# genome/bam-readcount

Measured on AMD Instinct MI355X. Metric: pileup base-events/sec, higher is better.
Workload: dtype u32+f32

## Files before the change

bam_readcount_amd/csrc/brc_engine.hip:

```cpp
#include <hip/hip_runtime.h>
#include <atomic>
#include <chrono>

#include <stdio.h>
#include <stdlib.h>
#include <string.h>

#include <algorithm>
#include <string>
#include <mutex>
#include <vector>

#include "brc_host.h"

namespace brc {

struct Counters {
    unsigned long long n_events, n_positions, w_sm, w_nm, w_lib;
    unsigned int n_indel_slots, n_xev;
    unsigned int xev_max, n_wave_reads;
    unsigned int n_wave_big, n_wave_huge;
    unsigned int n_literal, n_wave_eqx;
    unsigned int n_wave_eqx_big, pad_;
};
// ... 1797 lines not shown

static void* pinned_alloc(size_t n) {
    void* p = nullptr;
    if (hipHostMalloc(&p, n ? n : 1, hipHostMallocDefault) != hipSuccess) return nullptr;
    return p;
}
static void pinned_release(void* p) { (void)hipHostFree(p); }
static const HostAlloc kPinned = {pinned_alloc, pinned_release};

static std::atomic<uint64_t> g_dev_allocs{0}, g_dev_alloc_ns{0};
struct DBuf {
    void* p = nullptr; size_t cap = 0;
    size_t req = 0;
    hipError_t ensure(size_t bytes) {
        req = bytes;
        if (bytes <= cap) return hipSuccess;
        struct Tm { std::chrono::steady_clock::time_point t0 = std::chrono::steady_clock::now();
                    ~Tm() { g_dev_alloc_ns += (uint64_t)std::chrono::duration_cast<std::chrono::nanoseconds>(std::chrono::steady_clock::now() - t0).count(); ++g_dev_allocs; } } tm_;
        const bool regrow = p != nullptr;
        if (p) { (void)hipFree(p); p = nullptr; cap = 0; }
        size_t want = bytes + (regrow ? bytes / 2 : bytes / 8) + 256;
        hipError_t e = hipMalloc(&p, want);
        if (e != hipSuccess) { e = hipMalloc(&p, bytes); want = bytes; }
        if (e == hipSuccess) cap = want;
        return e;
    }
    void release() { if (p) (void)hipFree(p); p = nullptr; cap = 0; }
};

enum { T_ANNOTATE = 0, T_SCAN_ENDS, T_TILES, T_PILEUP, T_COUNT, T_INDEL_SCAN, T_INDEL_FILL, T_INDEL_REDUCE, T_N };
static const char* kKernelNames[BRC_NKERNEL] = {"k_annotate", "k_scan_ends", "k_tiles", "k_pileup", "k_xev_fold+finalize",
                                                "k_scan_indel", "k_indel_fill", "k_indel_reduce"};

#define HIPCHK(x) do { hipError_t _e = (x); if (_e != hipSuccess) { return hip_fail(_e, #x); } } while (0)

class HipBackend : public Backend {
    std::string err;
    int device = 0;
    hipStream_t stream = nullptr;
    enum { EV_RING = 32 };
    struct EvSet { hipEvent_t evt[T_N + 1]; hipEvent_t ev_indel[4]; };
    std::vector<EvSet> evsets;
    hipEvent_t* evt = nullptr;
    bool have_events = false;
    DevCfg c; DevIn in;
    int64_t ntiles = 0; uint64_t n_indel_cap = 0;
    std::vector<int64_t> lib_base;
    DBuf d_pos, d_flag, d_mapq, d_lib, d_lq, d_nc, d_co, d_so, d_qo, d_nm, d_sm, d_tags, d_cigar, d_seq, d_qual, d_ref, d_refcode;
    std::vector<uint16_t> h_wanted; bool has_wanted = false; DBuf d_wanted; std::vector<uint32_t> h_tilelist; DBuf d_tilelist;
    HBuf<Staged::WidePair> h_wpairs; unsigned wide_slices = 1;
    DBuf d_wpairs;
    DBuf d_bq, d_bqw, d_bqrow, d_pieceoff, d_pieces, d_rare, d_keyreach, d_libbase, d_reads, d_agg, d_rng, d_ncol, d_depth, d_slotid, d_si, d_sf, d_xev, d_xevc, d_xevn, d_unavail, d_cnt, d_cursor, d_ev, d_evraw, d_ievoff, d_iout, d_ctr, d_tilectr, d_part, d_wavelist, d_nc_k1;
    DBuf d_tlen, d_toff, d_text, d_tctx, d_total64, d_lastproc;
    DBuf d_xcnt, d_xend, d_xidx, d_xagg;
    HBuf<char> h_text[2]; HBuf<uint32_t> h_toff[2]; HBuf<uint32_t> h_total;
    hipStream_t stream2 = nullptr; hipEvent_t ev_text[2] = {nullptr, nullptr}, ev_lines = nullptr;
    hipStream_t stream3 = nullptr; hipEvent_t* ev_indel = nullptr; DBuf d_agg2;
    bool text_started[2] = {false, false}; uint64_t text_total[2] = {0, 0}; int64_t text_n[2] = {0, 0}; int text_slot = 0;
    Planes pl_last;
    enum { COMPACT_PIECES_PER_READ = 12 };
    bool compact_on = false; uint64_t compact_total = 0; bool compact_sized = false;
    bool wave_on = false;
    bool wave_big = false;
    enum { WAVE_FORM_BLOCKS = 768,
           WAVE_FORM_BLOCKS_BIG = 512,
           WAVE_FORM_BLOCKS_HUGE = 256 };
    bool wave_huge = false;
    bool wave_eqx = false; uint32_t s_max_ncigar = 0;
    bool cursor_on = false;
    unsigned long long h_steps[3] = {0, 0, 0};
    DBuf d_ccnt, d_coff, d_cpieces, d_crare, d_crng, d_ctot;
    HBuf<uint32_t> h_ncol, h_depth, h_slotid, h_si, h_unavail; HBuf<float> h_sf; HBuf<IndelOut> h_iout; HBuf<XAgg> h_xagg; HBuf<uint32_t> h_lastproc[2];
    std::vector<XAgg> xagg_compact;
    size_t xev_cap = 0;
    enum { XEV_SHARDS = 1024 };
    std::vector<IndelOut> iout_compact;
    Counters h_ctr;
    bool computed = false;
#ifdef BRC_CHECKED
    DBuf d_chk; ChkState h_chk;
    void chk_fill() {
        memset(&h_chk, 0, sizeof h_chk);
        auto set = [&](int b, const DBuf& d) { h_chk.ext[b].lo = (uint64_t)d.p; h_chk.ext[b].hi = (uint64_t)d.p + d.req; };
        set(CB_CIGAR, d_cigar); set(CB_SEQ, d_seq); set(CB_QUAL, d_qual); set(CB_REFCODE, d_refcode); set(CB_EB, d_bq); set(CB_BQW, d_bqw);
        set(CB_PIECES, d_pieces); set(CB_RARE, d_rare); set(CB_KEYREACH, d_keyreach); set(CB_READS, d_reads); set(CB_EVRAW, d_evraw); set(CB_CNT, d_cnt);
        set(CB_WANTED, d_wanted); set(CB_RNG, d_rng); set(CB_UNAVAIL, d_unavail); set(CB_TILELIST, d_tilelist); set(CB_NCOL, d_ncol); set(CB_DEPTH, d_depth);
        set(CB_SLOTID, d_slotid); set(CB_SI, d_si); set(CB_SF, d_sf); set(CB_XEV, d_xev); set(CB_XEVN, d_xevn); set(CB_TILECTR, d_tilectr);
        const bool cz = compact_on && compact_sized;
        set(CB_KP_PIECES, cz ? d_cpieces : d_pieces); set(CB_KP_RARE, cz ? d_crare : d_rare); set(CB_KP_RNG, cz ? d_crng : d_rng);
        if (const char* sh = getenv("BRC_CHECKED_SHRINK")) { const int b = atoi(sh); const char* cpos = strchr(sh, ':'); if (b >= 0 && b < CB_N && cpos) { const uint64_t by = strtoull(cpos + 1, nullptr, 10); ChkExt& x = h_chk.ext[b]; x.hi = x.hi - x.lo > by ? x.hi - by : x.lo; } }
// ... 20 lines not shown
        err = b;
        return e == hipErrorOutOfMemory ? BRC_E_NOMEM : BRC_E_HIP;
    }

  public:
    int init(int dev) {
        int n = 0;
        if (hipGetDeviceCount(&n) != hipSuccess || n <= 0) { err = "no HIP device visible"; return BRC_E_NODEVICE; }
        if (dev < 0 || dev >= n) { err = "device ordinal out of range"; return BRC_E_NODEVICE; }
        device = dev;
        HIPCHK(hipSetDevice(device));
        HIPCHK(hipStreamCreateWithFlags(&stream, hipStreamNonBlocking));
        { const int rc0 = ensure_evsets(1); if (rc0) return rc0; }
        HIPCHK(hipStreamCreateWithFlags(&stream2, hipStreamNonBlocking));
        HIPCHK(hipStreamCreateWithFlags(&stream3, hipStreamNonBlocking));
        {
            uint32_t* d_bad = nullptr; uint32_t bad = 0;
            HIPCHK(hipMalloc(&d_bad, sizeof(uint32_t)));
            HIPCHK(hipMemsetAsync(d_bad, 0, sizeof(uint32_t), stream));
            hipLaunchKernelGGL(k_divcheck, dim3((DIV_SMALL_N * DIV_SMALL_M + 255) / 256), dim3(256), 0, stream, d_bad);
            HIPCHK(hipMemcpyAsync(&bad, d_bad, sizeof(uint32_t), hipMemcpyDeviceToHost, stream));
            HIPCHK(hipStreamSynchronize(stream));
            (void)hipFree(d_bad);
            if (bad) { err = "this device's reciprocal does not give correctly rounded small-integer quotients (div_small self-check failed)"; return BRC_E_HIP; }
        }
        for (int i = 0; i < 2; ++i) { HIPCHK(hipEventCreateWithFlags(&ev_text[i], hipEventDisableTiming)); h_text[i].A = &kPinned; h_toff[i].A = &kPinned; }
        HIPCHK(hipEventCreateWithFlags(&ev_lines, hipEventDisableTiming));
        h_total.A = &kPinned;
        h_ncol.A = h_depth.A = h_slotid.A = h_si.A = h_unavail.A = &kPinned; h_sf.A = &kPinned; h_iout.A = &kPinned; h_xagg.A = &kPinned; h_wpairs.A = &kPinned; h_lastproc[0].A = h_lastproc[1].A = &kPinned;
        return BRC_OK;
    }
    ~HipBackend() override {
        (void)hipSetDevice(device);
        if (getenv("BRC_ENGINE_TIMING")) fprintf(stderr, "device buffers: %llu (re)allocations, %.3f s\n", (unsigned long long)g_dev_allocs.load(), (double)g_dev_alloc_ns.load() * 1e-9);
        DBuf* all[] = {&d_pos, &d_flag, &d_mapq, &d_lib, &d_lq, &d_nc, &d_co, &d_so, &d_qo, &d_nm, &d_sm, &d_tags, &d_cigar, &d_seq, &d_qual,
                       &d_ref, &d_refcode, &d_bq, &d_bqw, &d_bqrow, &d_pieceoff, &d_pieces, &d_rare, &d_keyreach, &d_libbase, &d_reads, &d_agg, &d_rng, &d_ncol, &d_depth, &d_slotid, &d_si, &d_sf, &d_xev, &d_xevc, &d_xevn, &d_unavail, &d_cnt,
                       &d_cursor, &d_ev, &d_evraw, &d_ievoff, &d_iout, &d_ctr, &d_tilectr, &d_part, &d_tlen, &d_toff, &d_text, &d_tctx, &d_total64, &d_lastproc, &d_xcnt, &d_xend, &d_xidx, &d_xagg, &d_wanted, &d_tilelist, &d_wavelist, &d_nc_k1, &d_wpairs};
        for (DBuf* b : all) b->release();
        d_ccnt.release(); d_coff.release(); d_cpieces.release(); d_crare.release(); d_crng.release(); d_ctot.release();
#ifdef BRC_CHECKED
        d_chk.release();
#endif
        for (int i = 0; i < 2; ++i) { h_text[i].destroy(); h_toff[i].destroy(); if (ev_text[i]) (void)hipEventDestroy(ev_text[i]); }
        h_total.destroy();
        if (ev_lines) (void)hipEventDestroy(ev_lines);
        if (stream2) (void)hipStreamDestroy(stream2);
        if (stream3) (void)hipStreamDestroy(stream3);
        d_agg2.release();
        h_ncol.destroy(); h_depth.destroy(); h_slotid.destroy(); h_si.destroy(); h_unavail.destroy(); h_sf.destroy(); h_iout.destroy(); h_xagg.destroy(); h_wpairs.destroy(); h_lastproc[0].destroy(); h_lastproc[1].destroy();
        if (w_init) { w_ncol.destroy(); w_depth.destroy(); w_slotid.destroy(); w_si.destroy(); w_unavail.destroy(); w_sf.destroy(); }
        for (EvSet& es : evsets) { for (int i = 0; i <= T_N; ++i) if (es.evt[i]) (void)hipEventDestroy(es.evt[i]); for (int i = 0; i < 4; ++i) if (es.ev_indel[i]) (void)hipEventDestroy(es.ev_indel[i]); }
        if (stream) (void)hipStreamDestroy(stream);
    }
    int ensure_evsets(size_t n) {
        while (evsets.size() < n) {
            EvSet es; memset(&es, 0, sizeof es);
            evsets.push_back(es);
            for (int i = 0; i <= T_N; ++i) HIPCHK(hipEventCreate(&evsets.back().evt[i]));
            for (int i = 0; i < 4; ++i) HIPCHK(hipEventCreate(&evsets.back().ev_indel[i]));
        }
        evt = evsets[0].evt; ev_indel = evsets[0].ev_indel; have_events = true;
        return BRC_OK;
    }
    const HostAlloc* host_alloc() override { return &kPinned; }
    const char* last_error() const override { return err.c_str(); }

    template <class T>
    int up(DBuf& d, const HBuf<T>& h, size_t n) {
        HIPCHK(d.ensure((n + 16) * sizeof(T)));
        if (n) HIPCHK(hipMemcpyAsync(d.p, h.p, n * sizeof(T), hipMemcpyHostToDevice, stream));
        return BRC_OK;
    }

    int up_arena(DBuf& d, const HBuf<uint8_t>& h, const std::vector<Staged::Seg>& segs, uint64_t total) {
        if (segs.empty()) return up(d, h, h.n);
        HIPCHK(d.ensure((size_t)total + 16));
        for (const Staged::Seg& g : segs) if (g.n) HIPCHK(hipMemcpyAsync((uint8_t*)d.p + g.off, g.p, (size_t)g.n, hipMemcpyHostToDevice, stream));
        return BRC_OK;
    }
    bool adopts_arenas() const override { return true; }

    int upload(const brc_config& cfg, const Staged& s, Geometry& g) override {
        HIPCHK(hipSetDevice(device));
        computed = false;
        memset(&c, 0, sizeof c);
        c.min_mapq = cfg.min_mapq; c.min_bq = cfg.min_bq; c.per_lib = cfg.per_lib; c.insertion_centric = cfg.insertion_centric;
        c.Lp = g.Lp; c.ref_len_check = cfg.ref_len_check; c.has_ref = g.ref != nullptr;
        g.PS = (g.P + 63) & ~(int64_t)63;
        c.beg0 = g.beg0; c.end = g.end; c.pos0 = g.pos0; c.P = g.P; c.PS = g.PS; c.ref_lo = g.ref_lo; c.ref_hi = g.ref_hi; c.ref_len = g.ref_len;
        c.n_reads = s.n; c.table_len = test_knob(TK_NO_TABLE) ? 0 : s.modal_len();
        c.n_pieces = s.n_pieces; lib_base = s.lib_base; c.max_lqseq = s.max_lqseq;
        c.ibucket_shift = indel_bucket_shift(s.n_indel_ops, c.P, c.Lp);
        if (const char* ib = test_knob(TK_IBUCKET_SHIFT)) { const int v = atoi(ib); if (v == 2 || v == 4 || v == 6) c.ibucket_shift = v; }
        choose_pack(s.max_lqseq, test_knob(TK_FLUSH_K) ? atoi(test_knob(TK_FLUSH_K)) : 0, test_knob(TK_PACK_LIM) ? atoi(test_knob(TK_PACK_LIM)) : 0, c.flush_k, c.pack_lim, c.pack_lim_lo, c.pack_shift);
// ... 94 lines not shown
        HIPCHK(d_ctr.ensure(sizeof(Counters))); HIPCHK(d_tilectr.ensure(((size_t)ntiles * Lp + 1) * sizeof(uint4)));
        in.iev_off = nullptr;
        if (n_indel_cap) {
            const size_t nbk = (size_t)indel_buckets(c);
            if ((rc = up(d_ievoff, s.iev_off, n))) return rc;
            in.iev_off = (const uint32_t*)d_ievoff.p;
            HIPCHK(d_cnt.ensure(nbk * 4 + 16)); HIPCHK(d_cursor.ensure(nbk * 4 + 16)); HIPCHK(d_evraw.ensure((n_indel_cap + 1) * sizeof(IndelEv)));
            HIPCHK(d_ev.ensure((n_indel_cap + 1) * sizeof(IndelEv))); HIPCHK(d_iout.ensure((n_indel_cap + 1) * sizeof(IndelOut)));
        }
        if (has_wanted && P) {
            HIPCHK(hipMemsetAsync(d_ncol.p, 0, Lp * P * 4, stream)); HIPCHK(hipMemsetAsync(d_depth.p, 0, Lp * P * 4, stream));
            HIPCHK(hipMemsetD32Async((hipDeviceptr_t)d_slotid.p, (int)((uint32_t)NB_NONE | ((uint32_t)NB_NONE << 8)), Lp * P, stream));
            HIPCHK(hipMemsetAsync(d_tilectr.p, 0, (size_t)ntiles * Lp * sizeof(uint4), stream));
        }
        HIPCHK(hipStreamSynchronize(stream));
        return BRC_OK;
    }

    template <class Op, bool INCL>
    int scan(const typename Op::T* src, typename Op::T* dst, int64_t n) { return scan_on<Op, INCL>(src, dst, n, stream, d_agg); }
    template <class Op, bool INCL>
    int scan_on(const typename Op::T* src, typename Op::T* dst, int64_t n, hipStream_t st, DBuf& scratch) {
        if (n <= 0) return BRC_OK;
        const int64_t nb = (n + SCAN_CHUNK - 1) / SCAN_CHUNK;
        typename Op::T* agg = (typename Op::T*)scratch.p;
        hipLaunchKernelGGL((k_scan_reduce<Op>), dim3((unsigned)nb), dim3(SCAN_T), 0, st, src, n, agg);
        hipLaunchKernelGGL((k_scan_aggregates<Op>), dim3(1), dim3(1024), 0, st, agg, nb);
        hipLaunchKernelGGL((k_scan_apply<Op, INCL>), dim3((unsigned)nb), dim3(SCAN_T), 0, st, src, dst, n, (const typename Op::T*)agg);
        HIPCHK(hipGetLastError());
        return BRC_OK;
    }

    int enqueue_pass(size_t set) {
        evt = evsets[set].evt; ev_indel = evsets[set].ev_indel;
        const int64_t n = c.n_reads, P = c.P; const int Lp = c.Lp;
        int rc;
        Counters* ctr = (Counters*)d_ctr.p;
        lists_host = false;
        HIPCHK(hipMemsetAsync(ctr, 0, sizeof(Counters), stream));
        HIPCHK(hipMemsetAsync(d_xevn.p, 0, (size_t)XEV_SHARDS * XEV_CTR_STRIDE * 4, stream));
        const bool indels = n_indel_cap > 0 && P > 0 && n > 0;
        const int64_t n_buckets = indel_buckets(c);
        if (indels) HIPCHK(hipMemsetAsync(d_cnt.p, 0, (size_t)n_buckets * 4, stream));
#ifdef BRC_CHECKED
        if (set == 0) { chk_fill(); HIPCHK(hipMemcpyAsync(d_chk.p, &h_chk, sizeof h_chk, hipMemcpyHostToDevice, stream)); HIPCHK(hipStreamSynchronize(stream)); }
#endif
        Planes pl = {(uint32_t*)d_ncol.p, (uint32_t*)d_depth.p, (uint32_t*)d_slotid.p, (uint32_t*)d_si.p, (float*)d_sf.p, (uint32_t*)d_unavail.p,
                     (XEv*)d_xev.p, (uint32_t*)d_xevn.p, (uint32_t)xev_cap, (uint32_t)XEV_SHARDS};
        pl_last = pl;
        const DRead* reads = (const DRead*)d_reads.p;
        HIPCHK(hipEventRecord(evt[T_ANNOTATE], stream));
        if (n > 0) {
            const int64_t rl = c.ref_hi - c.ref_lo;
            if (c.has_ref)
                hipLaunchKernelGGL(k_refcode, dim3((unsigned)(((rl + 2 * REFCODE_PAD + 15) / 16 + 255) / 256)), dim3(256), 0, stream, in.ref, (uint8_t*)d_refcode.p, rl);
            if (h_wpairs.n)
                hipLaunchKernelGGL(k_wide_rows, dim3((unsigned)((h_wpairs.n + 255) / 256), wide_slices), dim3(256), 0, stream, c, in, (const uint2*)d_wpairs.p, (uint32_t)h_wpairs.n, (uint16_t*)in.bqw);
            DevIn in_k1 = in;
            if (wave_on || cursor_on) {
                hipLaunchKernelGGL(k_pick_wave, dim3((unsigned)((n + 255) / 256)), dim3(256), 0, stream, c, in, (uint32_t*)d_nc_k1.p, (uint32_t*)d_wavelist.p, (uint32_t)n, &ctr->n_wave_reads, &ctr->n_wave_big, &ctr->n_wave_huge,
                                   wave_on ? 1 : 0, cursor_on ? 1 : 0, &ctr->n_literal, &ctr->n_wave_eqx, &ctr->n_wave_eqx_big);
                in_k1.n_cigar = (const uint32_t*)d_nc_k1.p;
            }
            {
#define BRC_LAUNCH_K1(OS, SH) hipLaunchKernelGGL((k_annotate_groups<OS, SH>), dim3((unsigned)((n + 255) / 256)), dim3(256), 0, stream, c, in_k1, (DRead*)d_reads.p, (const uint32_t*)d_pieceoff.p, \
                                   (Piece*)d_pieces.p, (PieceRare*)d_rare.p, (int2*)d_keyreach.p,                                                                               \
                                   (uint8_t*)in.eb, indels ? (IndelEv*)d_evraw.p : (IndelEv*)nullptr, (uint32_t*)d_cnt.p,                                    \
                                   in.cigar, in.qual, in.seq4, (const uint8_t*)d_refcode.p + REFCODE_PAD, has_wanted ? (const uint16_t*)d_wanted.p : (const uint16_t*)nullptr)
                if (Lp == 1) { if (c.pack_shift == 16) BRC_LAUNCH_K1(true, 16); else BRC_LAUNCH_K1(true, 12); }
                else { if (c.pack_shift == 16) BRC_LAUNCH_K1(false, 16); else BRC_LAUNCH_K1(false, 12); }
#undef BRC_LAUNCH_K1
                if (wave_on) {
                    const unsigned nb = (unsigned)std::min<int64_t>((n + 3) / 4, (int64_t)WAVE_FORM_BLOCKS);
#define BRC_LAUNCH_K1W(SH, MCAP, WAVES, GRID, LIST, STEP, COUNT) hipLaunchKernelGGL((k_annotate_wave<SH, MCAP, WAVES>), dim3(GRID), dim3(WAVES * 64), 0, stream, c, in, LIST, STEP, (const unsigned int*)(COUNT),     \
                                   (DRead*)d_reads.p, (const uint32_t*)d_pieceoff.p, (Piece*)d_pieces.p, (PieceRare*)d_rare.p, (int2*)d_keyreach.p,                                   \
                                   (uint8_t*)in.eb, indels ? (IndelEv*)d_evraw.p : (IndelEv*)nullptr, (uint32_t*)d_cnt.p,                                          \
                                   (const uint8_t*)d_refcode.p + REFCODE_PAD, has_wanted ? (const uint16_t*)d_wanted.p : (const uint16_t*)nullptr)
                    const uint32_t* const wl = (const uint32_t*)d_wavelist.p;
                    if (c.pack_shift == 16) BRC_LAUNCH_K1W(16, AW_MCAP, 4, nb, wl, 1, &ctr->n_wave_reads); else BRC_LAUNCH_K1W(12, AW_MCAP, 4, nb, wl, 1, &ctr->n_wave_reads);
                    if (wave_big) {
                        const unsigned nbb = (unsigned)std::min<int64_t>(n, (int64_t)WAVE_FORM_BLOCKS_BIG);
                        if (c.pack_shift == 16) BRC_LAUNCH_K1W(16, AW_MCAP_BIG, 1, nbb, wl + (n - 1), -1, &ctr->n_wave_big); else BRC_LAUNCH_K1W(12, AW_MCAP_BIG, 1, nbb, wl + (n - 1), -1, &ctr->n_wave_big);
                    }
                    if (wave_eqx) {
#define BRC_LAUNCH_K1E(SH, MCAP, WAVES, GRID, LIST, STEP, COUNT) hipLaunchKernelGGL((k_annotate_wave<SH, MCAP, WAVES, true>), dim3(GRID), dim3(WAVES * 64), 0, stream, c, in, LIST, STEP, (const unsigned int*)(COUNT),     \
                                   (DRead*)d_reads.p, (const uint32_t*)d_pieceoff.p, (Piece*)d_pieces.p, (PieceRare*)d_rare.p, (int2*)d_keyreach.p,                                   \
                                   (uint8_t*)in.eb, indels ? (IndelEv*)d_evraw.p : (IndelEv*)nullptr, (uint32_t*)d_cnt.p,                                          \
                                   (const uint8_t*)d_refcode.p + REFCODE_PAD, has_wanted ? (const uint16_t*)d_wanted.p : (const uint16_t*)nullptr)
                        if (c.pack_shift == 16) BRC_LAUNCH_K1E(16, AW_MCAP_EQX, 4, nb, wl + (3 * n + 48), 1, &ctr->n_wave_eqx); else BRC_LAUNCH_K1E(12, AW_MCAP_EQX, 4, nb, wl + (3 * n + 48), 1, &ctr->n_wave_eqx);
                        if (s_max_ncigar > (uint32_t)AW_MCAP_EQX) {
                            const unsigned nbe = (unsigned)std::min<int64_t>(n, (int64_t)WAVE_FORM_BLOCKS_BIG);
                            if (c.pack_shift == 16) BRC_LAUNCH_K1E(16, AW_MCAP_EQX_BIG, 1, nbe, wl + (4 * n + 47), -1, &ctr->n_wave_eqx_big); else BRC_LAUNCH_K1E(12, AW_MCAP_EQX_BIG, 1, nbe, wl + (4 * n + 47), -1, &ctr->n_wave_eqx_big);
                        }
#undef BRC_LAUNCH_K1E
                    }
                    if (wave_huge) {
                        const unsigned nbh = (unsigned)std::min<int64_t>(n, (int64_t)WAVE_FORM_BLOCKS_HUGE);
                        if (c.pack_shift == 16) BRC_LAUNCH_K1W(16, AW_MCAP_HUGE, 1, nbh, wl + (n + 16), 1, &ctr->n_wave_huge); else BRC_LAUNCH_K1W(12, AW_MCAP_HUGE, 1, nbh, wl + (n + 16), 1, &ctr->n_wave_huge);
                    }
#undef BRC_LAUNCH_K1W
                }
                if (cursor_on) {
                    const unsigned nbc = (unsigned)std::min<int64_t>((n + 63) / 64, 1024);
#define BRC_LAUNCH_K1C(SH) hipLaunchKernelGGL((k_annotate_cursor<SH>), dim3(nbc), dim3(64), 0, stream, c, in, (const uint32_t*)d_wavelist.p + (2 * (size_t)n + 32), (const unsigned int*)&ctr->n_literal,    \
                                   (DRead*)d_reads.p, (const uint32_t*)d_pieceoff.p, (Piece*)d_pieces.p, (PieceRare*)d_rare.p, (int2*)d_keyreach.p, (uint8_t*)in.eb,                     \
                                   indels ? (IndelEv*)d_evraw.p : (IndelEv*)nullptr, (uint32_t*)d_cnt.p, has_wanted ? (const uint16_t*)d_wanted.p : (const uint16_t*)nullptr)
                    if (c.pack_shift == 16) BRC_LAUNCH_K1C(16); else BRC_LAUNCH_K1C(12);
#undef BRC_LAUNCH_K1C
                }
            }
            if (c.per_lib) {
                HIPCHK(hipMemsetAsync(d_unavail.p, 0xff, (size_t)c.PS * 4, stream));
                hipLaunchKernelGGL(k_unavail, dim3((unsigned)((n + 255) / 256)), dim3(256), 0, stream, c, in, (uint32_t*)d_unavail.p);
            }
        } else if (c.per_lib && P > 0) HIPCHK(hipMemsetAsync(d_unavail.p, 0xff, (size_t)c.PS * 4, stream));
        HIPCHK(hipEventRecord(evt[T_SCAN_ENDS], stream));
#ifdef BRC_EXP_KNOBS
        static const bool indel_overlap = getenv("BRC_INDEL_OVERLAP") && atoi(getenv("BRC_INDEL_OVERLAP")) != 0;
#else
        const bool indel_overlap = false;
#endif
        auto launch_indel = [&](hipStream_t si, DBuf& scratch) -> int {
            HIPCHK(hipEventRecord(ev_indel[0], si));
            int r2;
            if ((r2 = scan_on<OpSumU32, false>((const uint32_t*)d_cnt.p, (uint32_t*)d_cursor.p, n_buckets, si, scratch))) return r2;
            HIPCHK(hipEventRecord(ev_indel[1], si));
            hipLaunchKernelGGL(k_indel_scatter, dim3((unsigned)((n_indel_cap + 255) / 256)), dim3(256), 0, si, c, (const IndelEv*)d_evraw.p, (int64_t)n_indel_cap,
                               (uint32_t*)d_cursor.p, (IndelEv*)d_ev.p);
            HIPCHK(hipEventRecord(ev_indel[2], si));
            hipLaunchKernelGGL(k_indel_reduce, dim3((unsigned)std::min<int64_t>((n_buckets + 255) / 256, 4096)), dim3(256), 0, si, c, in, reads,
                               (const uint32_t*)d_cnt.p, (const uint32_t*)d_cursor.p, n_buckets, (IndelEv*)d_ev.p, (const uint32_t*)d_unavail.p,
                               (IndelOut*)d_iout.p, ctr);
            HIPCHK(hipEventRecord(ev_indel[3], si));
            return BRC_OK;
        };
        if (indels && indel_overlap) {
            HIPCHK(hipStreamWaitEvent(stream3, evt[T_SCAN_ENDS], 0));
            if ((rc = launch_indel(stream3, d_agg2))) return rc;
        }
        const int64_t np_all = c.n_pieces;
        const int64_t trb = (np_all + TR_CHUNK - 1) / TR_CHUNK;
        if (np_all > 0 && ntiles > 0) {
            hipLaunchKernelGGL(k_reach_blockmax, dim3((unsigned)trb), dim3(TR_T), 0, stream, (const int2*)d_keyreach.p, np_all, (const int64_t*)d_libbase.p, Lp, (unsigned long long*)d_agg.p);
            hipLaunchKernelGGL((k_scan_aggregates<OpMaxU64>), dim3(1), dim3(1024), 0, stream, (unsigned long long*)d_agg.p, trb);
        }
        HIPCHK(hipEventRecord(evt[T_TILES], stream));
        for (int l = 0; l < Lp && ntiles > 0; ++l)
            if (lib_base[(size_t)l + 1] == lib_base[(size_t)l]) HIPCHK(hipMemsetAsync((uint2*)d_rng.p + (int64_t)l * ntiles, 0, (size_t)ntiles * sizeof(uint2), stream));
        if (np_all > 0 && ntiles > 0)
            hipLaunchKernelGGL(k_tiles_all, dim3((unsigned)trb), dim3(TR_T), 0, stream, c, (const int2*)d_keyreach.p, np_all, (const int64_t*)d_libbase.p, Lp,
                               (const unsigned long long*)d_agg.p, ntiles, (uint2*)d_rng.p);
        const int64_t n_listed = (int64_t)h_tilelist.size();
        if (has_wanted && n_listed > 0)
            hipLaunchKernelGGL(k_narrow_tiles, dim3((unsigned)((n_listed * Lp + 255) / 256)), dim3(256), 0, stream, (const uint16_t*)d_wanted.p, (const uint32_t*)d_tilelist.p, n_listed, ntiles, Lp, c.pos0,
                               (uint2*)d_rng.p, (const int2*)d_keyreach.p);
        const uint4* kp_pieces = (const uint4*)d_pieces.p; const PieceRare* kp_rare = (const PieceRare*)d_rare.p; const uint2* kp_rng = (const uint2*)d_rng.p;
        if (compact_on && ntiles > 0 && np_all > 0) {
            const size_t nslot = (size_t)ntiles * (size_t)Lp;
            HIPCHK(d_ccnt.ensure((nslot + 2) * 4)); HIPCHK(d_coff.ensure((nslot + 2) * 4)); HIPCHK(d_crng.ensure((nslot + 1) * sizeof(uint2))); HIPCHK(d_ctot.ensure(24));
            HIPCHK(hipMemsetAsync(d_ctot.p, 0, 24, stream));
            HIPCHK(hipMemsetAsync((uint32_t*)d_ccnt.p + nslot, 0, 4, stream));
            const dim3 cg((unsigned)((ntiles + 3) / 4), (unsigned)Lp);
            const bool by_read = Lp == 1 && !(test_knob(TK_COMPACT) && atoi(test_knob(TK_COMPACT)) == 2);
            if (by_read) {
                HIPCHK(hipMemsetAsync(d_ccnt.p, 0, nslot * 4, stream));
                hipLaunchKernelGGL(k_count_piece_tiles, dim3((unsigned)((np_all + 255) / 256)), dim3(256), 0, stream, c, (const uint4*)d_pieces.p, np_all, (uint32_t*)d_ccnt.p);
            }
            else
            hipLaunchKernelGGL((k_compact_tiles<true>), cg, dim3(256), 0, stream, c, (const uint4*)d_pieces.p, (const PieceRare*)d_rare.p, (const uint2*)d_rng.p, ntiles,
                               (uint32_t*)d_ccnt.p, (const uint32_t*)nullptr, (uint4*)nullptr, (PieceRare*)nullptr, (uint2*)nullptr, (unsigned long long*)d_ctot.p);
            if ((rc = scan<OpSumU32, false>((const uint32_t*)d_ccnt.p, (uint32_t*)d_coff.p, (int64_t)nslot + 1))) return rc;
            const bool first_pass = !compact_sized;
            if (!compact_sized) {
                uint32_t tot = 0;
                HIPCHK(hipMemcpyAsync(&tot, (const uint32_t*)d_coff.p + nslot, 4, hipMemcpyDeviceToHost, stream));
                HIPCHK(hipMemcpyAsync(h_steps, d_ctot.p, 16, hipMemcpyDeviceToHost, stream));
                HIPCHK(hipStreamSynchronize(stream));
                compact_total = tot; compact_sized = true;
                HIPCHK(d_cpieces.ensure(((size_t)compact_total + 4) * sizeof(Piece))); HIPCHK(d_crare.ensure(((size_t)compact_total + 2) * sizeof(PieceRare)));
            }
            if (by_read)
                hipLaunchKernelGGL(k_compact_reads, dim3((unsigned)((ntiles + 4 * CR_GROUP - 1) / (4 * CR_GROUP))), dim3(256), 0, stream, c, (const uint4*)d_pieces.p, (const PieceRare*)d_rare.p, (const uint2*)d_rng.p, (const uint32_t*)d_pieceoff.p, (const int2*)d_keyreach.p, ntiles,
                                   (const uint32_t*)d_coff.p, (uint4*)d_cpieces.p, (PieceRare*)d_crare.p, (uint2*)d_crng.p, (unsigned long long*)d_ctot.p);
            else
            hipLaunchKernelGGL((k_compact_tiles<false>), cg, dim3(256), 0, stream, c, (const uint4*)d_pieces.p, (const PieceRare*)d_rare.p, (const uint2*)d_rng.p, ntiles,
                               (uint32_t*)d_ccnt.p, (const uint32_t*)d_coff.p, (uint4*)d_cpieces.p, (PieceRare*)d_crare.p, (uint2*)d_crng.p, (unsigned long long*)d_ctot.p);
            if (by_read && first_pass) {
                HIPCHK(hipMemcpyAsync(h_steps, d_ctot.p, 24, hipMemcpyDeviceToHost, stream));
                HIPCHK(hipStreamSynchronize(stream));
                if (h_steps[2]) { err = "tile compaction: a tile holds more live read segments than the pass over the segments counted for it"; return BRC_E_HIP; }
            }
            kp_pieces = (const uint4*)d_cpieces.p; kp_rare = (const PieceRare*)d_crare.p; kp_rng = (const uint2*)d_crng.p;
#ifdef BRC_CHECKED
            {
                HIPCHK(hipStreamSynchronize(stream));
                ChkState seen; HIPCHK(hipMemcpy(&seen, d_chk.p, sizeof seen, hipMemcpyDeviceToHost));
                chk_fill(); ChkState upd = h_chk; upd.count = seen.count; upd.kernel = seen.kernel; upd.site = seen.site; upd.buf = seen.buf; upd.addr = seen.addr; upd.bytes = seen.bytes; upd.unit = seen.unit; upd.piece = seen.piece;
                HIPCHK(hipMemcpy(d_chk.p, &upd, sizeof upd, hipMemcpyHostToDevice));
            }
#endif
        }
        HIPCHK(hipEventRecord(evt[T_PILEUP], stream));
        if (ntiles > 0) {
            unsigned nwg = (unsigned)(((has_wanted ? n_listed : ntiles) + PILEUP_WAVES - 1) / PILEUP_WAVES);
            nwg = (nwg + 7u) & ~7u;
#ifdef BRC_EXP_KNOBS
            static const unsigned dyn_lds = getenv("BRC_PILEUP_LDS_PAD") ? (unsigned)atoi(getenv("BRC_PILEUP_LDS_PAD")) : 0u;
#else
            const unsigned dyn_lds = 0u;
#endif
#define BRC_LAUNCH_KP(W, SH) hipLaunchKernelGGL((k_pileup2<W, SH>), dim3(nwg, (unsigned)Lp), dim3(PILEUP_WAVES * 64), dyn_lds, stream, c, in, kp_pieces, kp_rare, \
                               kp_rng, ntiles, pl, (uint4*)d_tilectr.p, in.eb, in.bqw, (const uint32_t*)d_unavail.p,                                                     \
                               (const uint8_t*)d_refcode.p + REFCODE_PAD, (const uint16_t*)d_wanted.p, (const uint32_t*)d_tilelist.p, n_listed)
            if (has_wanted) { if (n_listed > 0) { if (c.pack_shift == 16) BRC_LAUNCH_KP(true, 16); else BRC_LAUNCH_KP(true, 12); } }
            else { if (c.pack_shift == 16) BRC_LAUNCH_KP(false, 16); else BRC_LAUNCH_KP(false, 12); }
#undef BRC_LAUNCH_KP
        }
        HIPCHK(hipEventRecord(evt[T_COUNT], stream));
        if (ntiles > 0) {
            const int64_t nxb = ntiles * Lp;
            HIPCHK(hipMemsetAsync(d_xcnt.p, 0, (size_t)nxb * 4, stream));
            hipLaunchKernelGGL(k_xev_compact, dim3((unsigned)XEV_SHARDS), dim3(256), 0, stream, (const XEv*)d_xev.p, (const uint32_t*)d_xevn.p, (uint32_t)xev_cap,
                               (uint32_t)XEV_SHARDS, (XEv*)d_xevc.p, ctr, (uint32_t*)d_xcnt.p, Lp);
            if ((rc = scan<OpSumU32, false>((const uint32_t*)d_xcnt.p, (uint32_t*)d_xend.p, nxb))) return rc;
            hipLaunchKernelGGL(k_xev_scatter, dim3(256), dim3(256), 0, stream, (const XEv*)d_xevc.p, (const Counters*)ctr, (uint32_t*)d_xend.p, (uint32_t*)d_xidx.p, Lp);
            hipLaunchKernelGGL(k_xev_fold, dim3((unsigned)std::min<int64_t>((nxb + 255) / 256, 2048)), dim3(256), 0, stream, (const XEv*)d_xevc.p, (uint32_t*)d_xcnt.p, (uint32_t*)d_xend.p, nxb,
                               (uint32_t*)d_xidx.p, (XAgg*)d_xagg.p);
        }
        if (P > 0) {
            const unsigned nb = (unsigned)std::min<int64_t>(((Lp > 1 ? P / 4 : ntiles) + 255) / 256 + 1, Lp > 1 ? 4096 : 256);
            hipLaunchKernelGGL(k_finalize, dim3(nb), dim3(256), 0, stream, c, (const uint32_t*)d_ncol.p, (const uint4*)d_tilectr.p, (int64_t)ntiles * Lp,
                               (unsigned long long*)d_part.p);
            hipLaunchKernelGGL(k_finalize_sum, dim3(1), dim3(256), 0, stream, (const unsigned long long*)d_part.p, (int)nb, ctr);
        }
        HIPCHK(hipEventRecord(evt[T_INDEL_SCAN], stream));
        if (indels && !indel_overlap) { if ((rc = launch_indel(stream, d_agg))) return rc; }
        if (indels && indel_overlap) HIPCHK(hipStreamWaitEvent(stream, ev_indel[3], 0));
        HIPCHK(hipEventRecord(evt[T_N], stream));
        HIPCHK(hipGetLastError());
        return BRC_OK;
    }
    int finish_passes(bool* again) {
        HIPCHK(hipMemcpyAsync(&h_ctr, d_ctr.p, sizeof(Counters), hipMemcpyDeviceToHost, stream));
        HIPCHK(hipStreamSynchronize(stream));
        *again = false;
#ifdef BRC_CHECKED
        { const int rcc = chk_report(); if (rcc) return rcc; }
#endif
        if ((size_t)h_ctr.xev_max > xev_cap) {
            xev_cap = (size_t)h_ctr.xev_max * 2;
            HIPCHK(d_xev.ensure(((size_t)XEV_SHARDS * xev_cap + 1) * sizeof(XEv))); HIPCHK(d_xevc.ensure(((size_t)XEV_SHARDS * xev_cap + 1) * sizeof(XEv)));
            HIPCHK(d_xidx.ensure(((size_t)XEV_SHARDS * xev_cap + 1) * 4)); HIPCHK(d_xagg.ensure(((size_t)XEV_SHARDS * xev_cap + 1) * sizeof(XAgg)));
            *again = true;
        }
        return BRC_OK;
    }
    int add_timing(size_t set, brc_timing* t) {
        const bool indels = n_indel_cap > 0 && c.P > 0 && c.n_reads > 0;
        const EvSet& es = evsets[set]; float ms = 0;
        for (int i = 0; i < T_INDEL_SCAN; ++i) { HIPCHK(hipEventElapsedTime(&ms, es.evt[i], es.evt[i + 1])); t->ms[i] += ms; }
        if (indels) for (int i = 0; i < 3; ++i) { HIPCHK(hipEventElapsedTime(&ms, es.ev_indel[i], es.ev_indel[i + 1])); t->ms[T_INDEL_SCAN + i] += ms; }
        HIPCHK(hipEventElapsedTime(&ms, es.evt[0], es.evt[T_N])); t->total_ms += ms;
        return BRC_OK;
    }
    int compute(brc_timing* t) override {
        HIPCHK(hipSetDevice(device));
        for (;;) {
            int rc = enqueue_pass(0); if (rc) return rc;
            bool again = false;
            if ((rc = finish_passes(&again))) return rc;
// ... 230 lines not shown
```

bam_readcount_amd/csrc/brc_host.h:

```cpp
#ifndef BRC_HOST_H
#define BRC_HOST_H

#include <stddef.h>
#include <stdint.h>
#include <string.h>

#include <string>
#include <vector>

#include "../../include/brc.h"
#include "brc_core.h"

namespace brc {

struct HostAlloc {
    void* (*alloc)(size_t bytes);
    void (*release)(void* p);
};

template <class T>
struct HBuf {
    T* p = nullptr;
    size_t n = 0, cap = 0;
    const HostAlloc* A = nullptr;
// ... 105 lines not shown
    virtual void list_sizes(uint64_t* n_xev, uint64_t* n_indel_slots) { *n_xev = 0; *n_indel_slots = 0; }
    virtual int device_view(brc_device_view* out) {
        HostPlanes hp;
        const int rc = fetch(&hp, true); if (rc) return rc;
        out->memory = BRC_MEM_HOST; out->device = 0;
        out->ncol = hp.ncol; out->depth = hp.depth; out->slotid = hp.slotid; out->si = hp.si; out->sf = hp.sf; out->unavail = hp.unavail;
        out->xagg = hp.xagg; out->n_xagg = hp.n_xagg;
        return BRC_OK;
    }
    virtual int device_indels(const Staged& s, const Geometry& g, brc_device_indels* out) {
        HostPlanes hp;
        const int rc = fetch(&hp, false); if (rc) return rc;
        out->memory = BRC_MEM_HOST; out->device = 0;
        out->slots = hp.n_indel ? hp.indel : nullptr; out->n_slots = (uint64_t)hp.n_indel;
        out->seq4 = s.seq4.p; out->seq_off = s.seq_off.p; out->l_qseq = s.l_qseq.p; out->n_reads = s.n;
        out->ref = g.ref ? g.ref + g.ref_lo : nullptr;
        return BRC_OK;
    }
    virtual int counts(uint64_t* n_events, uint64_t* n_positions) = 0;
    virtual void piece_steps(uint64_t* ranged, uint64_t* walked) { *ranged = 0; *walked = 0; }
    virtual const char* last_error() const = 0;
};

Backend* make_backend(const brc_config& cfg, int* err);
void* backend_host_alloc(size_t bytes);
void backend_host_free(void* p);
const char* backend_kind();
const char* backend_kernel_name(int k);

void expand_slots(const HostPlanes& hp, int Lp, int64_t P, int64_t PS, uint32_t* istat, float* fstat);

unsigned effective_cpus();

enum TestKnob { TK_NO_TABLE = 0, TK_FLUSH_K, TK_PACK_LIM, TK_FORCE_DOM, TK_IBUCKET_SHIFT, TK_XEV_CAP, TK_DEVICE_TEXT_LIMIT, TK_FORMAT_THREADS, TK_FORMAT_CHUNK, TK_COMPACT, TK_WAVE_FORM, TK_N };
const char* test_knob(int which);

int fmt_f2(char* out, float v);
int fmt_u32(char* out, uint32_t v);

}
#endif
```

bam_readcount_amd/csrc/brc_knobs.cpp:

```cpp
#include <stdlib.h>

#include "brc_host.h"

namespace brc {
#ifdef BRC_TEST_KNOBS
const char* test_knob(int which) {
    static const char* const kNames[TK_N] = {"BRC_NO_TABLE", "BRC_FLUSH_K", "BRC_PACK_LIM", "BRC_FORCE_DOM", "BRC_IBUCKET_SHIFT", "BRC_XEV_CAP", "BRC_DEVICE_TEXT_LIMIT", "BRC_FORMAT_THREADS", "BRC_FORMAT_CHUNK", "BRC_COMPACT_TILES", "BRC_WAVE_FORM"};
    return (which >= 0 && which < TK_N) ? getenv(kNames[which]) : nullptr;
}
#else
const char* test_knob(int) { return nullptr; }
#endif
}
```

Measured before the change: 338.4 billion.

## Run unavail, wide-rows, finalize and indel passes on a side stream DAG

Restructures each compute pass into a two-stream dependency graph. The unavail and wide-row input kernels run on a side stream concurrently with annotate and tiling, joined before pileup by an event. After pileup, finalize and the indel scan/scatter/reduce run on the side stream in parallel with xev compact/fold on the main stream, and the xcnt memset moves up front. This targets idle time from serial small kernels, at the cost of extra events and cross-stream waits, plus a serial fallback knob.

```diff
diff --git a/bam_readcount_amd/csrc/brc_engine.hip b/bam_readcount_amd/csrc/brc_engine.hip
--- a/bam_readcount_amd/csrc/brc_engine.hip
+++ b/bam_readcount_amd/csrc/brc_engine.hip
@@ -1853,6 +1853,10 @@
 static const char* kKernelNames[BRC_NKERNEL] = {"k_annotate", "k_scan_ends", "k_tiles", "k_pileup", "k_xev_fold+finalize",
                                                 "k_scan_indel", "k_indel_fill", "k_indel_reduce"};
 
+#ifndef BRC_PASS_INDEL_LATE
+#define BRC_PASS_INDEL_LATE 0
+#endif
+
 #define HIPCHK(x) do { hipError_t _e = (x); if (_e != hipSuccess) { return hip_fail(_e, #x); } } while (0)
 
 class HipBackend : public Backend {
@@ -1860,7 +1864,8 @@
     int device = 0;
     hipStream_t stream = nullptr;
     enum { EV_RING = 32 };
-    struct EvSet { hipEvent_t evt[T_N + 1]; hipEvent_t ev_indel[4]; };
+    enum { D_START = 0, D_PILEIN, D_SIDE_END, D_N };
+    struct EvSet { hipEvent_t evt[T_N + 1]; hipEvent_t ev_indel[4]; hipEvent_t ev_dep[D_N]; };
     std::vector<EvSet> evsets;
     hipEvent_t* evt = nullptr;
     bool have_events = false;
@@ -1876,7 +1881,7 @@
     DBuf d_xcnt, d_xend, d_xidx, d_xagg;
     HBuf<char> h_text[2]; HBuf<uint32_t> h_toff[2]; HBuf<uint32_t> h_total;
     hipStream_t stream2 = nullptr; hipEvent_t ev_text[2] = {nullptr, nullptr}, ev_lines = nullptr;
-    hipStream_t stream3 = nullptr; hipEvent_t* ev_indel = nullptr; DBuf d_agg2;
+    hipStream_t stream3 = nullptr; hipEvent_t* ev_indel = nullptr; hipEvent_t* ev_dep = nullptr; DBuf d_agg2;
     bool text_started[2] = {false, false}; uint64_t text_total[2] = {0, 0}; int64_t text_n[2] = {0, 0}; int text_slot = 0;
     Planes pl_last;
     enum { COMPACT_PIECES_PER_READ = 12 };
@@ -1963,6 +1968,8 @@
     }
     ~HipBackend() override {
         (void)hipSetDevice(device);
+        if (stream3) (void)hipStreamSynchronize(stream3);
+        if (stream) (void)hipStreamSynchronize(stream);
         if (getenv("BRC_ENGINE_TIMING")) fprintf(stderr, "device buffers: %llu (re)allocations, %.3f s\n", (unsigned long long)g_dev_allocs.load(), (double)g_dev_alloc_ns.load() * 1e-9);
         DBuf* all[] = {&d_pos, &d_flag, &d_mapq, &d_lib, &d_lq, &d_nc, &d_co, &d_so, &d_qo, &d_nm, &d_sm, &d_tags, &d_cigar, &d_seq, &d_qual,
                        &d_ref, &d_refcode, &d_bq, &d_bqw, &d_bqrow, &d_pieceoff, &d_pieces, &d_rare, &d_keyreach, &d_libbase, &d_reads, &d_agg, &d_rng, &d_ncol, &d_depth, &d_slotid, &d_si, &d_sf, &d_xev, &d_xevc, &d_xevn, &d_unavail, &d_cnt,
@@ -1980,7 +1987,8 @@
         d_agg2.release();
         h_ncol.destroy(); h_depth.destroy(); h_slotid.destroy(); h_si.destroy(); h_unavail.destroy(); h_sf.destroy(); h_iout.destroy(); h_xagg.destroy(); h_wpairs.destroy(); h_lastproc[0].destroy(); h_lastproc[1].destroy();
         if (w_init) { w_ncol.destroy(); w_depth.destroy(); w_slotid.destroy(); w_si.destroy(); w_unavail.destroy(); w_sf.destroy(); }
-        for (EvSet& es : evsets) { for (int i = 0; i <= T_N; ++i) if (es.evt[i]) (void)hipEventDestroy(es.evt[i]); for (int i = 0; i < 4; ++i) if (es.ev_indel[i]) (void)hipEventDestroy(es.ev_indel[i]); }
+        for (EvSet& es : evsets) { for (int i = 0; i <= T_N; ++i) if (es.evt[i]) (void)hipEventDestroy(es.evt[i]); for (int i = 0; i < 4; ++i) if (es.ev_indel[i]) (void)hipEventDestroy(es.ev_indel[i]);
+                                   for (int i = 0; i < D_N; ++i) if (es.ev_dep[i]) (void)hipEventDestroy(es.ev_dep[i]); }
         if (stream) (void)hipStreamDestroy(stream);
     }
     int ensure_evsets(size_t n) {
@@ -1989,8 +1997,9 @@
             evsets.push_back(es);
             for (int i = 0; i <= T_N; ++i) HIPCHK(hipEventCreate(&evsets.back().evt[i]));
             for (int i = 0; i < 4; ++i) HIPCHK(hipEventCreate(&evsets.back().ev_indel[i]));
-        }
-        evt = evsets[0].evt; ev_indel = evsets[0].ev_indel; have_events = true;
+            for (int i = 0; i < D_N; ++i) HIPCHK(hipEventCreateWithFlags(&evsets.back().ev_dep[i], hipEventDisableTiming));
+        }
+        evt = evsets[0].evt; ev_indel = evsets[0].ev_indel; ev_dep = evsets[0].ev_dep; have_events = true;
         return BRC_OK;
     }
     const HostAlloc* host_alloc() override { return &kPinned; }
@@ -2151,30 +2160,65 @@
     }
 
     int enqueue_pass(size_t set) {
-        evt = evsets[set].evt; ev_indel = evsets[set].ev_indel;
+        const int rc = enqueue_pass_dag(set);
+        if (rc) { (void)hipStreamSynchronize(stream3); (void)hipStreamSynchronize(stream); }
+        return rc;
+    }
+    int enqueue_pass_dag(size_t set) {
+        evt = evsets[set].evt; ev_indel = evsets[set].ev_indel; ev_dep = evsets[set].ev_dep;
         const int64_t n = c.n_reads, P = c.P; const int Lp = c.Lp;
         int rc;
         Counters* ctr = (Counters*)d_ctr.p;
         lists_host = false;
+#ifdef BRC_CHECKED
+        const bool serial = true;
+#else
+        const bool serial = test_knob(TK_SERIAL_PASS) && atoi(test_knob(TK_SERIAL_PASS)) != 0;
+#endif
+        const hipStream_t side = serial ? stream : stream3;
+        const bool indels = n_indel_cap > 0 && P > 0 && n > 0;
+        const int64_t n_buckets = indel_buckets(c);
+        const DRead* reads = (const DRead*)d_reads.p;
+        const bool side_inputs = !serial && ((c.per_lib && P > 0) || (n > 0 && h_wpairs.n > 0));
+        auto launch_inputs = [&](hipStream_t st) -> int {
+            if (c.per_lib && P > 0) HIPCHK(hipMemsetAsync(d_unavail.p, 0xff, (size_t)c.PS * 4, st));
+            if (c.per_lib && n > 0) hipLaunchKernelGGL(k_unavail, dim3((unsigned)((n + 255) / 256)), dim3(256), 0, st, c, in, (uint32_t*)d_unavail.p);
+            if (n > 0 && h_wpairs.n)
+                hipLaunchKernelGGL(k_wide_rows, dim3((unsigned)((h_wpairs.n + 255) / 256), wide_slices), dim3(256), 0, st, c, in, (const uint2*)d_wpairs.p, (uint32_t)h_wpairs.n, (uint16_t*)in.bqw);
+            return BRC_OK;
+        };
+        auto launch_finalize = [&]() -> int {
+            if (P > 0) {
+                const unsigned nb = (unsigned)std::min<int64_t>(((Lp > 1 ? P / 4 : ntiles) + 255) / 256 + 1, Lp > 1 ? 4096 : 256);
+                hipLaunchKernelGGL(k_finalize, dim3(nb), dim3(256), 0, side, c, (const uint32_t*)d_ncol.p, (const uint4*)d_tilectr.p, (int64_t)ntiles * Lp,
+                                   (unsigned long long*)d_part.p);
+                hipLaunchKernelGGL(k_finalize_sum, dim3(1), dim3(256), 0, side, (const unsigned long long*)d_part.p, (int)nb, ctr);
+            }
+            return BRC_OK;
+        };
+        if (side_inputs) {
+            HIPCHK(hipEventRecord(ev_dep[D_START], stream));
+            HIPCHK(hipStreamWaitEvent(side, ev_dep[D_START], 0));
+            if ((rc = launch_inputs(side))) return rc;
+            HIPCHK(hipEventRecord(ev_dep[D_PILEIN], side));
+        }
         HIPCHK(hipMemsetAsync(ctr, 0, sizeof(Counters), stream));
         HIPCHK(hipMemsetAsync(d_xevn.p, 0, (size_t)XEV_SHARDS * XEV_CTR_STRIDE * 4, stream));
-        const bool indels = n_indel_cap > 0 && P > 0 && n > 0;
-        const int64_t n_buckets = indel_buckets(c);
         if (indels) HIPCHK(hipMemsetAsync(d_cnt.p, 0, (size_t)n_buckets * 4, stream));
+        if (ntiles > 0) HIPCHK(hipMemsetAsync(d_xcnt.p, 0, (size_t)(ntiles * Lp) * 4, stream));
 #ifdef BRC_CHECKED
         if (set == 0) { chk_fill(); HIPCHK(hipMemcpyAsync(d_chk.p, &h_chk, sizeof h_chk, hipMemcpyHostToDevice, stream)); HIPCHK(hipStreamSynchronize(stream)); }
 #endif
         Planes pl = {(uint32_t*)d_ncol.p, (uint32_t*)d_depth.p, (uint32_t*)d_slotid.p, (uint32_t*)d_si.p, (float*)d_sf.p, (uint32_t*)d_unavail.p,
                      (XEv*)d_xev.p, (uint32_t*)d_xevn.p, (uint32_t)xev_cap, (uint32_t)XEV_SHARDS};
         pl_last = pl;
-        const DRead* reads = (const DRead*)d_reads.p;
         HIPCHK(hipEventRecord(evt[T_ANNOTATE], stream));
+        if (n > 0 && c.has_ref) {
+            const int64_t rl = c.ref_hi - c.ref_lo;
+            hipLaunchKernelGGL(k_refcode, dim3((unsigned)(((rl + 2 * REFCODE_PAD + 15) / 16 + 255) / 256)), dim3(256), 0, stream, in.ref, (uint8_t*)d_refcode.p, rl);
+        }
+        if (!side_inputs && (rc = launch_inputs(stream))) return rc;
         if (n > 0) {
-            const int64_t rl = c.ref_hi - c.ref_lo;
-            if (c.has_ref)
-                hipLaunchKernelGGL(k_refcode, dim3((unsigned)(((rl + 2 * REFCODE_PAD + 15) / 16 + 255) / 256)), dim3(256), 0, stream, in.ref, (uint8_t*)d_refcode.p, rl);
-            if (h_wpairs.n)
-                hipLaunchKernelGGL(k_wide_rows, dim3((unsigned)((h_wpairs.n + 255) / 256), wide_slices), dim3(256), 0, stream, c, in, (const uint2*)d_wpairs.p, (uint32_t)h_wpairs.n, (uint16_t*)in.bqw);
             DevIn in_k1 = in;
             if (wave_on || cursor_on) {
                 hipLaunchKernelGGL(k_pick_wave, dim3((unsigned)((n + 255) / 256)), dim3(256), 0, stream, c, in, (uint32_t*)d_nc_k1.p, (uint32_t*)d_wavelist.p, (uint32_t)n, &ctr->n_wave_reads, &ctr->n_wave_big, &ctr->n_wave_huge,
@@ -2228,34 +2272,25 @@
 #undef BRC_LAUNCH_K1C
                 }
             }
-            if (c.per_lib) {
-                HIPCHK(hipMemsetAsync(d_unavail.p, 0xff, (size_t)c.PS * 4, stream));
-                hipLaunchKernelGGL(k_unavail, dim3((unsigned)((n + 255) / 256)), dim3(256), 0, stream, c, in, (uint32_t*)d_unavail.p);
-            }
-        } else if (c.per_lib && P > 0) HIPCHK(hipMemsetAsync(d_unavail.p, 0xff, (size_t)c.PS * 4, stream));
+        }
         HIPCHK(hipEventRecord(evt[T_SCAN_ENDS], stream));
-#ifdef BRC_EXP_KNOBS
-        static const bool indel_overlap = getenv("BRC_INDEL_OVERLAP") && atoi(getenv("BRC_INDEL_OVERLAP")) != 0;
-#else
-        const bool indel_overlap = false;
-#endif
-        auto launch_indel = [&](hipStream_t si, DBuf& scratch) -> int {
-            HIPCHK(hipEventRecord(ev_indel[0], si));
+        auto launch_indel = [&](DBuf& scratch) -> int {
+            HIPCHK(hipEventRecord(ev_indel[0], side));
             int r2;
-            if ((r2 = scan_on<OpSumU32, false>((const uint32_t*)d_cnt.p, (uint32_t*)d_cursor.p, n_buckets, si, scratch))) return r2;
-            HIPCHK(hipEventRecord(ev_indel[1], si));
-            hipLaunchKernelGGL(k_indel_scatter, dim3((unsigned)((n_indel_cap + 255) / 256)), dim3(256), 0, si, c, (const IndelEv*)d_evraw.p, (int64_t)n_indel_cap,
+            if ((r2 = scan_on<OpSumU32, false>((const uint32_t*)d_cnt.p, (uint32_t*)d_cursor.p, n_buckets, side, scratch))) return r2;
+            HIPCHK(hipEventRecord(ev_indel[1], side));
+            hipLaunchKernelGGL(k_indel_scatter, dim3((unsigned)((n_indel_cap + 255) / 256)), dim3(256), 0, side, c, (const IndelEv*)d_evraw.p, (int64_t)n_indel_cap,
                                (uint32_t*)d_cursor.p, (IndelEv*)d_ev.p);
-            HIPCHK(hipEventRecord(ev_indel[2], si));
-            hipLaunchKernelGGL(k_indel_reduce, dim3((unsigned)std::min<int64_t>((n_buckets + 255) / 256, 4096)), dim3(256), 0, si, c, in, reads,
+            HIPCHK(hipEventRecord(ev_indel[2], side));
+            hipLaunchKernelGGL(k_indel_reduce, dim3((unsigned)std::min<int64_t>((n_buckets + 255) / 256, 4096)), dim3(256), 0, side, c, in, reads,
                                (const uint32_t*)d_cnt.p, (const uint32_t*)d_cursor.p, n_buckets, (IndelEv*)d_ev.p, (const uint32_t*)d_unavail.p,
                                (IndelOut*)d_iout.p, ctr);
-            HIPCHK(hipEventRecord(ev_indel[3], si));
+            HIPCHK(hipEventRecord(ev_indel[3], side));
             return BRC_OK;
         };
-        if (indels && indel_overlap) {
-            HIPCHK(hipStreamWaitEvent(stream3, evt[T_SCAN_ENDS], 0));
-            if ((rc = launch_indel(stream3, d_agg2))) return rc;
+        if (!serial && indels && !BRC_PASS_INDEL_LATE) {
+            HIPCHK(hipStreamWaitEvent(side, evt[T_SCAN_ENDS], 0));
+            if ((rc = launch_indel(d_agg2))) return rc;
         }
         const int64_t np_all = c.n_pieces;
         const int64_t trb = (np_all + TR_CHUNK - 1) / TR_CHUNK;
@@ -2319,6 +2354,7 @@
             }
 #endif
         }
+        if (side_inputs) HIPCHK(hipStreamWaitEvent(stream, ev_dep[D_PILEIN], 0));
         HIPCHK(hipEventRecord(evt[T_PILEUP], stream));
         if (ntiles > 0) {
             unsigned nwg = (unsigned)(((has_wanted ? n_listed : ntiles) + PILEUP_WAVES - 1) / PILEUP_WAVES);
@@ -2336,9 +2372,14 @@
 #undef BRC_LAUNCH_KP
         }
         HIPCHK(hipEventRecord(evt[T_COUNT], stream));
+        if (!serial) {
+            HIPCHK(hipStreamWaitEvent(side, evt[T_COUNT], 0));
+            if ((rc = launch_finalize())) return rc;
+            if (indels && BRC_PASS_INDEL_LATE) { if ((rc = launch_indel(d_agg2))) return rc; }
+            HIPCHK(hipEventRecord(ev_dep[D_SIDE_END], side));
+        }
         if (ntiles > 0) {
             const int64_t nxb = ntiles * Lp;
-            HIPCHK(hipMemsetAsync(d_xcnt.p, 0, (size_t)nxb * 4, stream));
             hipLaunchKernelGGL(k_xev_compact, dim3((unsigned)XEV_SHARDS), dim3(256), 0, stream, (const XEv*)d_xev.p, (const uint32_t*)d_xevn.p, (uint32_t)xev_cap,
                                (uint32_t)XEV_SHARDS, (XEv*)d_xevc.p, ctr, (uint32_t*)d_xcnt.p, Lp);
             if ((rc = scan<OpSumU32, false>((const uint32_t*)d_xcnt.p, (uint32_t*)d_xend.p, nxb))) return rc;
@@ -2346,15 +2387,10 @@
             hipLaunchKernelGGL(k_xev_fold, dim3((unsigned)std::min<int64_t>((nxb + 255) / 256, 2048)), dim3(256), 0, stream, (const XEv*)d_xevc.p, (uint32_t*)d_xcnt.p, (uint32_t*)d_xend.p, nxb,
                                (uint32_t*)d_xidx.p, (XAgg*)d_xagg.p);
         }
-        if (P > 0) {
-            const unsigned nb = (unsigned)std::min<int64_t>(((Lp > 1 ? P / 4 : ntiles) + 255) / 256 + 1, Lp > 1 ? 4096 : 256);
-            hipLaunchKernelGGL(k_finalize, dim3(nb), dim3(256), 0, stream, c, (const uint32_t*)d_ncol.p, (const uint4*)d_tilectr.p, (int64_t)ntiles * Lp,
-                               (unsigned long long*)d_part.p);
-            hipLaunchKernelGGL(k_finalize_sum, dim3(1), dim3(256), 0, stream, (const unsigned long long*)d_part.p, (int)nb, ctr);
-        }
+        if (serial && (rc = launch_finalize())) return rc;
         HIPCHK(hipEventRecord(evt[T_INDEL_SCAN], stream));
-        if (indels && !indel_overlap) { if ((rc = launch_indel(stream, d_agg))) return rc; }
-        if (indels && indel_overlap) HIPCHK(hipStreamWaitEvent(stream, ev_indel[3], 0));
+        if (serial && indels) { if ((rc = launch_indel(d_agg))) return rc; }
+        if (!serial) HIPCHK(hipStreamWaitEvent(stream, ev_dep[D_SIDE_END], 0));
         HIPCHK(hipEventRecord(evt[T_N], stream));
         HIPCHK(hipGetLastError());
         return BRC_OK;
diff --git a/bam_readcount_amd/csrc/brc_host.h b/bam_readcount_amd/csrc/brc_host.h
--- a/bam_readcount_amd/csrc/brc_host.h
+++ b/bam_readcount_amd/csrc/brc_host.h
@@ -161,7 +161,7 @@
 
 unsigned effective_cpus();
 
-enum TestKnob { TK_NO_TABLE = 0, TK_FLUSH_K, TK_PACK_LIM, TK_FORCE_DOM, TK_IBUCKET_SHIFT, TK_XEV_CAP, TK_DEVICE_TEXT_LIMIT, TK_FORMAT_THREADS, TK_FORMAT_CHUNK, TK_COMPACT, TK_WAVE_FORM, TK_N };
+enum TestKnob { TK_NO_TABLE = 0, TK_FLUSH_K, TK_PACK_LIM, TK_FORCE_DOM, TK_IBUCKET_SHIFT, TK_XEV_CAP, TK_DEVICE_TEXT_LIMIT, TK_FORMAT_THREADS, TK_FORMAT_CHUNK, TK_COMPACT, TK_WAVE_FORM, TK_SERIAL_PASS, TK_N };
 const char* test_knob(int which);
 
 int fmt_f2(char* out, float v);
diff --git a/bam_readcount_amd/csrc/brc_knobs.cpp b/bam_readcount_amd/csrc/brc_knobs.cpp
--- a/bam_readcount_amd/csrc/brc_knobs.cpp
+++ b/bam_readcount_amd/csrc/brc_knobs.cpp
@@ -5,7 +5,7 @@
 namespace brc {
 #ifdef BRC_TEST_KNOBS
 const char* test_knob(int which) {
-    static const char* const kNames[TK_N] = {"BRC_NO_TABLE", "BRC_FLUSH_K", "BRC_PACK_LIM", "BRC_FORCE_DOM", "BRC_IBUCKET_SHIFT", "BRC_XEV_CAP", "BRC_DEVICE_TEXT_LIMIT", "BRC_FORMAT_THREADS", "BRC_FORMAT_CHUNK", "BRC_COMPACT_TILES", "BRC_WAVE_FORM"};
+    static const char* const kNames[TK_N] = {"BRC_NO_TABLE", "BRC_FLUSH_K", "BRC_PACK_LIM", "BRC_FORCE_DOM", "BRC_IBUCKET_SHIFT", "BRC_XEV_CAP", "BRC_DEVICE_TEXT_LIMIT", "BRC_FORMAT_THREADS", "BRC_FORMAT_CHUNK", "BRC_COMPACT_TILES", "BRC_WAVE_FORM", "BRC_SERIAL_PASS"};
     return (which >= 0 && which < TK_N) ? getenv(kNames[which]) : nullptr;
 }
 #else
```

Result: no change. 341.4 billion (median of 6 runs) (+0.9%).
